# ucsdarclab/diffco

Measured on AMD Instinct MI355X. Metric: million collision-score+grad evals/sec, 7-DoF FK-kernel, 2k supports, higher is better.
Workload: dtype f32

## Files before the change

### diffco_amd/csrc/score_kernel.h

```cpp
#pragma once
#include <hip/hip_runtime.h>
#include <type_traits>
#include <stdint.h>
#include "fk_device.h"

namespace dcx {

enum { KF_RQ2 = 0,
       KF_POLY1 = 1,
       KF_GEN = 2 };

enum { MODE_SCORE = 0,
       MODE_GRAD_ROW = 1,
       MODE_GRAD_UP = 2 };

struct ScoreArgs {
    const float* rows;
    const float* centre;
    const FkProg* fk;
    const float* q;
    const float* upstream;
    float* score;
    float* grad;
    int64_t B;
// ... 125 lines not shown
#ifndef DCX_PAIR2_LOADS
#define DCX_PAIR2_LOADS 1
#endif
#ifndef DCX_LOAD_GROUPS
#define DCX_LOAD_GROUPS 1
#endif

template <int KF, bool CLAMPED = false>
__device__ __forceinline__ void kernel_eval(float d2, const ScoreArgs& a, float& val, float& g) {
    if constexpr (KF == KF_RQ2) {
        const float t = fmaf(0.5f * a.kp0, d2, 1.0f);
        const float u = __builtin_amdgcn_rcpf(t);
        val = u * u;
        g = (-2.0f * a.kp0) * (val * u);
    } else if constexpr (KF == KF_POLY1) {
        const float d2c = CLAMPED ? d2 : fmaxf(d2, 1e-30f);
        const float ri = __builtin_amdgcn_rsqf(d2c);
        val = d2c * ri;
        g = ri;
    } else {
        if (a.kind == DCX_K_RQ) {
            const float p = a.kp1;
            const float t = fmaf(a.kp0 / p, d2, 1.0f);
            val = powf(t, -p);
            g = (-2.0f * a.kp0) * val * __builtin_amdgcn_rcpf(t);
        } else if (a.kind == DCX_K_POLY) {
            const int k = (int)a.kp0;
            const float ie = 1.0f / a.kp1;
            const float d2c = fmaxf(d2, 1e-30f);
            const float ri = __builtin_amdgcn_rsqf(d2c);
            const float r = d2c * ri;
            float rk2 = (k >= 2) ? 1.0f : ri;
            for (int i = 2; i < k; ++i) rk2 *= r;
            if (k & 1) {
                val = rk2 * d2c * ie;
                g = (float)k * rk2 * ie;
            } else {
                const float lg = 0.5f * logf(d2c);
                val = rk2 * d2c * lg * ie;
                g = rk2 * fmaf((float)k, lg, 1.0f) * ie;
            }
        } else {
            const float ie2 = 1.0f / (a.kp0 * a.kp0);
            const float v2 = fmaf(d2, ie2, 1.0f);
            const float rv = __builtin_amdgcn_rsqf(v2);
            val = v2 * rv;
            g = rv * ie2;
        }
    }
}

template <int KF>
__device__ __forceinline__ float d2_seed(const ScoreArgs& a) {
    if constexpr (KF == KF_RQ2) return a.kp0;
    else return 0.0f;
}
template <int KF>
inline constexpr float kGradScale = (KF == KF_RQ2) ? -4.0f : 1.0f;
template <int KF, bool CLAMPED = false>
__device__ __forceinline__ void sweep_eval(float t, const ScoreArgs& a, float& val, float& g) {
    if constexpr (KF == KF_RQ2) {
        const float u = __builtin_amdgcn_rcpf(t);
        val = u * u;
        g = val * u;
    } else {
        kernel_eval<KF, CLAMPED>(t, a, val, g);
    }
}

struct LdsPlan {
    int fk, q, x, g, f, red, total;
};
__host__ __device__ inline LdsPlan lds_plan(int dof, int d_fk, int frame_floats, int red_slots, int acc_floats,
                                            bool alias_xg = false) {
    LdsPlan p;
    p.x = 0;
    p.g = alias_xg ? p.x : p.x + 64 * d_fk;
    p.red = p.x;
    const int end_xg = p.g + 64 * d_fk;
    const int end_red = p.red + (red_slots < 1 ? 1 : red_slots) * acc_floats * 64;
    p.q = end_xg > end_red ? end_xg : end_red;
    p.f = p.q + ((64 * dof + 3) & ~3);
    p.fk = p.f + 64 * frame_floats;
    p.total = p.fk;
    return p;
}

#ifndef DCX_MINW_SLACK
#define DCX_MINW_SLACK 0
#endif
constexpr int sweep_min_waves(int D, int CC, int KF, bool QT = false) {
    if (QT) return 4;
    const int need = 3 * D + 2 * CC + 16 + DCX_MINW_SLACK + (KF == 2 ? 40 : 0);
    return need <= 64 ? 8 : need <= 72 ? 7 : need <= 80 ? 6 : need <= 96 ? 5 : need <= 128 ? 4 : need <= 168 ? 3 : need <= 256 ? 2 : 1;
}

__device__ __forceinline__ int fresh_lane() {
    int l = (int)__builtin_amdgcn_mbcnt_hi(~0u, __builtin_amdgcn_mbcnt_lo(~0u, 0u));
    asm volatile("" : "+v"(l));
    return l;
}

template <class Args>
__device__ __forceinline__ const __attribute__((address_space(4))) Args& reload_kernargs() {
    auto p = (const __attribute__((address_space(4))) Args*)__builtin_amdgcn_kernarg_segment_ptr();
    asm volatile("" : "+s"(p));
    return *p;
}
__device__ __forceinline__ const __attribute__((address_space(4))) ScoreArgs& reload_args() { return reload_kernargs<ScoreArgs>(); }
#define DCX_COPY_DH(dst, src)          \
    do {                               \
        (dst).prog = (src).prog;       \
        (dst).n_dwords = (src).n_dwords; \
        (dst).n_steps = (src).n_steps; \
        (dst).end0 = (src).end0;       \
        (dst).n_chains = (src).n_chains; \
        (dst).pt = (src).pt;           \
        (dst).bare = (src).bare;       \
        (dst).real = (src).real;       \
        (dst).n_pt = (src).n_pt;       \
        (dst).shared_q = (src).shared_q; \
    } while (0)

__device__ __forceinline__ void row_opaque(float& u, float& v) { asm volatile("" : "+v"(u), "+v"(v)); }

#ifndef DCX_XF_TAU
#define DCX_XF_TAU 0.01f
#endif
#ifndef DCX_XF_FLUSH
#define DCX_XF_FLUSH 64
#endif

constexpr bool xf_applies(int D, int CC, int KF) {
    const int used = D + CC + (CC > 1 ? 1 : 0);
    const int parts = (4 * used <= (CC > 1 ? DCX_P0_MAX_MULTI : DCX_P0_MAX_SINGLE)) ? 0 : (used + 37) / 38;
    return (KF == KF_POLY1 || KF == KF_RQ2) && used + 1 <= 38 && parts <= 1;
}
constexpr bool spare_applies(int D, int CC, int KF) {
    return CC == 1 && (D % 4) == 0 && D >= 4 && D <= 12 && (KF == KF_POLY1 || KF == KF_RQ2) && D + 4 <= (D + 2 + 3) / 4 * 4;
}
constexpr bool p2_applies(int D, int CC, int KF) {
    return DCX_PAIR2 && DCX_PAIR2_LOADS && CC == 1 && (D % 2) == 0 && D <= DCX_PAIR2_MAX_D && 4 * (D + 1) <= DCX_P0_MAX_SINGLE &&
           (KF == KF_RQ2 || KF == KF_POLY1);
}

template <int D, int KF, int CC, int MODE, bool XF = false, int NACC = 0, bool NS = false, bool SP = false>
__device__ __forceinline__ void sweep_rows(const ScoreArgs& a, const float (&x_in)[D], const float (&up)[CC], int j0, int j1,
                                           float (&sc)[CC], float (&gx)[D]) {
    static_assert(!NS || (CC > 1 && MODE == MODE_GRAD_UP), "NS: the gradient sweep of a multi-class model");
    static_assert(!SP || (XF && spare_applies(D, CC, KF) && xf_applies(D, CC, KF)), "the spare form: expanded, one class, D = 4, 8, 12");
    float x[D];
    float e_sp = 0.0f, tot_sp = 0.0f;
    int col_sp = 0;
    if constexpr (SP) {
        const int c = a.spare - 1;
        e_sp = x_in[D - 1];
#pragma unroll
        for (int k = 0; k + 1 < D; ++k) {
            e_sp = (k == c) ? x_in[k] : e_sp;
            x[k] = (k == c) ? x_in[D - 1] : x_in[k];
        }
        x[D - 1] = 0.0f;
        col_sp = c;
        asm volatile("" : "+v"(col_sp));
    } else {
#pragma unroll
        for (int k = 0; k < D; ++k) x[k] = x_in[k];
    }
    using L = RowLayout<D, CC>;
    constexpr bool GRAD = (MODE != MODE_SCORE);
    v2f gx2[D / 2 + 1];
#pragma unroll
    for (int k = 0; k < D / 2 + 1; ++k) gx2[k] = v2f{0.0f, 0.0f};
    cfloat_ptr rows = (cfloat_ptr)(uintptr_t)a.rows;
    if constexpr (SP) {
        uint64_t rp = (uint64_t)(uintptr_t)a.rows;
        asm volatile("" : "+s"(rp));
        rows = (cfloat_ptr)(uintptr_t)rp;
    }
    constexpr int USED_DIRECT = D + CC + (CC > 1 ? 1 : 0);
    constexpr bool XFA = XF && xf_applies(D, CC, KF);
    constexpr int USED = SP ? D + 4 : USED_DIRECT + (XFA ? 1 : 0);
    constexpr int RSTRIDE = L::RS;
    constexpr int PARTS = SP ? 0 : (4 * USED <= (CC > 1 ? DCX_P0_MAX_MULTI : DCX_P0_MAX_SINGLE)) ? 0 : (USED + 37) / 38;
    constexpr bool SC2 = (CC > 1 && PARTS == 1);
    v2f sc2[CC / 2 + 1];
#pragma unroll
    for (int i = 0; i < CC / 2 + 1; ++i) sc2[i] = v2f{0.0f, 0.0f};
    auto add_scores = [&](auto weight_of, float val) __attribute__((always_inline)) {
        if constexpr (NS) {
            (void)val;
        } else if constexpr (SC2) {
            const v2f v2 = {val, val};
#pragma unroll
            for (int c = 0; c + 1 < CC; c += 2) sc2[c / 2] = __builtin_elementwise_fma(v2f{weight_of(c), weight_of(c + 1)}, v2, sc2[c / 2]);
            if constexpr (CC & 1) sc[CC - 1] = fmaf(weight_of(CC - 1), val, sc[CC - 1]);
#pragma unroll
            for (int c = 0; c + 1 < CC; c += 2) asm volatile("" : "+v"(sc2[c / 2]));
            if constexpr (CC & 1) asm volatile("" : "+v"(sc[CC - 1]));
        } else {
#pragma unroll
            for (int c = 0; c < CC; ++c) sc[c] = fmaf(weight_of(c), val, sc[c]);
        }
    };

    v2f xm[D / 2 + 1], ga[D / 2 + 1];
    float xm_tail = 0.0f, ga_tail = 0.0f, xx = 0.0f, thr = 1e-30f, asum = 0.0f;
    if constexpr (XFA) {
#pragma unroll
        for (int k = 0; k < D; ++k) xx = fmaf(x[k], x[k], xx);
        if constexpr (SP) xx = fmaf(e_sp, e_sp, xx);
        thr = fmaxf(DCX_XF_TAU * xx, 1e-30f);
#pragma unroll
        for (int k = 0; k + 1 < D; k += 2) {
            xm[k / 2] = v2f{-2.0f * x[k], -2.0f * x[k + 1]};
            ga[k / 2] = v2f{0.0f, 0.0f};
        }
        if constexpr (D & 1) xm_tail = -2.0f * x[D - 1];
        if constexpr (SP) xm[D / 2 - 1].y = 1.0f;
    }
    auto d2_x = [&](const auto& r) __attribute__((always_inline)) -> float {
        constexpr int NA = NACC > 0 ? NACC : DCX_D2_ACCS(D);
        v2f acc[NA];
        if constexpr (SP) acc[0] = v2f{xx, 0.0f};
        else acc[0] = v2f{xx + r[L::SS_OFF], 0.0f};
#pragma unroll
        for (int i = 1; i < NA; ++i) acc[i] = v2f{0.0f, 0.0f};
#pragma unroll
        for (int k = 0; k + 1 < D; k += 2) {
            const v2f rv = {r[k], r[k + 1]};
            acc[(k / 2) % NA] = __builtin_elementwise_fma(xm[k / 2], rv, acc[(k / 2) % NA]);
        }
#pragma unroll
        for (int i = 1; i < NA; ++i) acc[0] += acc[i];
        float d2 = acc[0].x + acc[0].y;
        if constexpr (D & 1) d2 = fmaf(xm_tail, r[D - 1], d2);
        if constexpr (KF == KF_POLY1) return fmaxf(d2, thr);
        else return d2;
    };
    auto coef_of = [&](const auto& r, float g) __attribute__((always_inline)) -> float {
        if constexpr (MODE == MODE_GRAD_ROW) {
            return g * r[CC > 1 ? L::WSUM_OFF : L::W_OFF];
        } else {
            float wb = 0.0f;
#pragma unroll
            for (int c = 0; c < CC; ++c) wb = fmaf(up[c], r[L::W_OFF + c], wb);
            return g * wb;
        }
    };
    auto apply_x = [&](const auto& r, float d2c, auto sign, bool keep) __attribute__((always_inline)) {
        constexpr int SIGN = decltype(sign)::value;
        float val, g;
        sweep_eval<KF, true>(d2c, a, val, g);
        if constexpr (PARTS == 1) row_opaque(val, g);
        constexpr bool SCORE_BY_COEF = (KF == KF_POLY1 && CC == 1 && MODE == MODE_GRAD_ROW);
        if constexpr (!SCORE_BY_COEF) {
            if constexpr (SIGN < 0) val = keep ? -val : 0.0f;
            add_scores([&](int c) __attribute__((always_inline)) { return r[L::W_OFF + c]; }, val);
        }
        if constexpr (GRAD) {
            float coef = coef_of(r, g);
            if constexpr (PARTS == 1) asm volatile("" : "+v"(coef));
            if constexpr (SIGN < 0) coef = keep ? -coef : 0.0f;
            if constexpr (SCORE_BY_COEF) sc[0] = fmaf(coef, d2c, sc[0]);
            const v2f c2 = {coef, coef};
#pragma unroll
            for (int k = 0; k + 1 < D; k += 2) {
                v2f rv = {r[k], r[k + 1]};
                if constexpr (SP) {
                    if (k == D - 2) rv = v2f{r[D + 2], r[D + 3]};
                }
                ga[k / 2] = __builtin_elementwise_fma(c2, rv, ga[k / 2]);
            }
            if constexpr (D & 1) ga_tail = fmaf(coef, r[D - 1], ga_tail);
            if constexpr (!SP) asum += coef;
        }
    };
    auto pair_x = [&](const auto& r) __attribute__((always_inline)) -> float {
        const float d2 = d2_x(r);
        apply_x(r, d2, std::integral_constant<int, 1>{}, true);
        return d2;
    };
    auto fix_near = [&](const auto& r, float d2c) __attribute__((always_inline)) {
        const bool nr = d2c <= thr;
        apply_x(r, d2c, std::integral_constant<int, -1>{}, nr);
        const v2f mh = {-0.5f, -0.5f};
        v2f dacc = {0.0f, 0.0f};
#pragma unroll
        for (int k = 0; k + 1 < D; k += 2) {
            const v2f rv = {r[k], r[k + 1]};
            v2f dk = xm[k / 2] * mh - rv;
            if constexpr (SP) {
                if (k == D - 2) dk.y = e_sp;
            }
            dacc = __builtin_elementwise_fma(dk, dk, dacc);
        }
        float d2d = dacc.x + dacc.y;
        if constexpr (D & 1) {
            const float dl_tail = -0.5f * xm_tail - r[D - 1];
            d2d = fmaf(dl_tail, dl_tail, d2d);
        }
        float val, g;
        kernel_eval<KF>(d2d, a, val, g);
        val = nr ? val : 0.0f;
        if constexpr (!NS) {
#pragma unroll
            for (int c = 0; c < CC; ++c) sc[c] = fmaf(r[L::W_OFF + c], val, sc[c]);
        }
        if constexpr (GRAD) {
            const float cd = nr ? -coef_of(r, g) : 0.0f;
            const v2f cd2 = {cd, cd};
#pragma unroll
            for (int k = 0; k + 1 < D; k += 2) {
                const v2f rv = {r[k], r[k + 1]};
                if (SP && k == D - 2) {
                    ga[k / 2].x = fmaf(cd, fmaf(xm[k / 2].x, -0.5f, -rv.x), ga[k / 2].x);
                    tot_sp -= cd;
                } else {
                    ga[k / 2] = __builtin_elementwise_fma(cd2, xm[k / 2] * mh - rv, ga[k / 2]);
                }
            }
            if constexpr (D & 1) ga_tail = fmaf(cd, -0.5f * xm_tail - r[D - 1], ga_tail);
        }
    };
    auto stage_x = [&](const auto& r0, const auto& r1) __attribute__((always_inline)) {
        if constexpr (KF != KF_POLY1) {
            (void)pair_x(r0);
            (void)pair_x(r1);
            return;
        }
        const auto m0 = __builtin_amdgcn_ballot_w64(pair_x(r0) <= thr);
        const auto m1 = __builtin_amdgcn_ballot_w64(pair_x(r1) <= thr);
        if (__builtin_expect((m0 | m1) != 0, 0)) {
            fix_near(r0, d2_x(r0));
            fix_near(r1, d2_x(r1));
        }
    };
    auto single_x = [&](const auto& r0) __attribute__((always_inline)) {
        if constexpr (KF != KF_POLY1) {
            (void)pair_x(r0);
            return;
        }
        if (__builtin_expect(__builtin_amdgcn_ballot_w64(pair_x(r0) <= thr) != 0, 0)) fix_near(r0, d2_x(r0));
    };
    auto flush_x = [&]() __attribute__((always_inline)) {
        if constexpr (XFA && GRAD) {
            if constexpr (SP) asum = ga[D / 2 - 1].y;
            const v2f ah = {0.5f * asum, 0.5f * asum};
#pragma unroll
            for (int k = 0; k + 1 < D; k += 2) ga[k / 2] = __builtin_elementwise_fma(xm[k / 2], ah, ga[k / 2]);
            if constexpr (D & 1) ga_tail = fmaf(xm_tail, 0.5f * asum, ga_tail);
            if constexpr (SP) {
                tot_sp += asum;
                ga[D / 2 - 1].y = 0.0f;
            }
            asum = 0.0f;
        }
    };
    auto pair = [&](const float (&r)[L::RS]) __attribute__((always_inline)) {
        float dl[D];
        float d2;
        v2f dp[D / 2 + 1];
        {
            constexpr int NA = DCX_D2_ACCS(D);
            v2f acc[NA];
            acc[0] = v2f{d2_seed<KF>(a), 0.0f};
#pragma unroll
            for (int i = 1; i < NA; ++i) acc[i] = v2f{0.0f, 0.0f};
#pragma unroll
            for (int k = 0; k + 1 < D; k += 2) {
                const v2f xv = {x[k], x[k + 1]};
                const v2f rv = {r[k], r[k + 1]};
                dp[k / 2] = xv - rv;
                acc[(k / 2) % NA] = __builtin_elementwise_fma(dp[k / 2], dp[k / 2], acc[(k / 2) % NA]);
            }
#pragma unroll
            for (int i = 1; i < NA; ++i) acc[0] += acc[i];
            d2 = acc[0].x + acc[0].y;
            if constexpr (D & 1) {
                dl[D - 1] = x[D - 1] - r[D - 1];
                d2 = fmaf(dl[D - 1], dl[D - 1], d2);
            }
        }
        float val, g;
        sweep_eval<KF>(d2, a, val, g);
        if constexpr (!NS) {
#pragma unroll
            for (int c = 0; c < CC; ++c) sc[c] = fmaf(r[L::W_OFF + c], val, sc[c]);
        }
        if constexpr (GRAD) {
            float coef;
            if constexpr (MODE == MODE_GRAD_ROW) {
                coef = g * r[CC > 1 ? L::WSUM_OFF : L::W_OFF];
            } else {
                float wb = 0.0f;
#pragma unroll
                for (int c = 0; c < CC; ++c) wb = fmaf(up[c], r[L::W_OFF + c], wb);
                coef = g * wb;
            }
            const v2f c2 = {coef, coef};
#pragma unroll
            for (int k = 0; k + 1 < D; k += 2) gx2[k / 2] = __builtin_elementwise_fma(c2, dp[k / 2], gx2[k / 2]);
            if constexpr (D & 1) gx[D - 1] = fmaf(coef, dl[D - 1], gx[D - 1]);
        }
    };
    constexpr bool P2 = !XF && p2_applies(D, CC, KF);
    static_assert(!P2 || PARTS == 0, "pair2: whole rows in the four-row budget");
    v2f gp[P2 ? D : 1];
    v2f scp = {0.0f, 0.0f};
    if constexpr (P2) {
#pragma unroll
        for (int k = 0; k < D; ++k) gp[k] = v2f{0.0f, 0.0f};
    }
    auto pair2 = [&](const float (&b)[2 * L::RS]) __attribute__((always_inline)) {
        v2f dk[D];
        v2f acc = {d2_seed<KF>(a), d2_seed<KF>(a)};
#pragma unroll
        for (int k = 0; k < D; ++k) {
            const v2f xv = {x[k], x[k]};
            const v2f rv = {b[2 * k], b[2 * k + 1]};
            dk[k] = xv - rv;
            acc = __builtin_elementwise_fma(dk[k], dk[k], acc);
        }
        v2f val, g;
        if constexpr (KF == KF_RQ2) {
            const v2f u = {__builtin_amdgcn_rcpf(acc.x), __builtin_amdgcn_rcpf(acc.y)};
            val = u * u;
            g = val * u;
        } else {
            const v2f d2c = {fmaxf(acc.x, 1e-30f), fmaxf(acc.y, 1e-30f)};
            g = v2f{__builtin_amdgcn_rsqf(d2c.x), __builtin_amdgcn_rsqf(d2c.y)};
            val = d2c * g;
        }
        const v2f w2 = {b[2 * L::W_OFF], b[2 * L::W_OFF + 1]};
        scp = __builtin_elementwise_fma(w2, val, scp);
        if constexpr (GRAD) {
            v2f coef = g * w2;
            if constexpr (MODE != MODE_GRAD_ROW) coef = coef * v2f{up[0], up[0]};
#pragma unroll
            for (int k = 0; k < D; ++k) gp[k] = __builtin_elementwise_fma(coef, dk[k], gp[k]);
        }
    };
    constexpr int USED4 = (USED + 3) / 4 * 4;
    static_assert(USED4 <= L::RS, "the row stride covers whole groups of four");
    constexpr int NLOAD = DCX_LOAD_GROUPS ? USED4 : USED;
#ifdef DCX_EXP_NO_LOADS
    int exp_real_loads = 4;
#endif
    auto load_row = [&](float (&dst)[L::RS], int j) __attribute__((always_inline)) {
        cfloat_ptr r = rows + (size_t)j * RSTRIDE;
#ifdef DCX_EXP_NO_LOADS
        if (exp_real_loads <= 0) {
#pragma unroll
            for (int e = 0; e < NLOAD; ++e) asm volatile("" : "+s"(dst[e]));
            return;
        }
        --exp_real_loads;
#endif
#pragma unroll
        for (int e = 0; e < NLOAD; ++e) {
            if (SP && e == D + 1) continue;
            dst[e] = r[e];
        }
    };

    static_assert(!XFA || PARTS <= 1, "expanded form: whole rows only");
    if constexpr (P2 && DCX_PAIR2_LOADS) {
    if (j0 < j1) {
        constexpr int R2 = 2 * L::RS;
        float ab[R2], cd[R2];
        auto load2 = [&](float (&dst)[R2], int j) __attribute__((always_inline)) {
            cfloat_ptr r = rows + (size_t)j * RSTRIDE;
#pragma unroll
            for (int e = 0; e < R2; ++e) dst[e] = r[e];
        };
        auto body2 = [&](const float (&b)[R2]) __attribute__((always_inline)) {
#pragma unroll
            for (int e = 2 * USED; e < R2; ++e) asm volatile("" ::"s"(b[e]));
            pair2(b);
        };
        const int j1e = (j1 + 1) & ~1;
        const int jl = j1e - 2;
        load2(ab, j0);
        int j = j0;
        for (; j + 3 < j1e; j += 4) {
            __builtin_amdgcn_s_waitcnt(0xC07F);
            __builtin_amdgcn_sched_barrier(0);
            load2(cd, j + 2);
            __builtin_amdgcn_sched_barrier(0);
            body2(ab);
            __builtin_amdgcn_sched_barrier(0);
            __builtin_amdgcn_s_waitcnt(0xC07F);
            __builtin_amdgcn_sched_barrier(0);
            load2(ab, (j + 4 < j1e) ? j + 4 : jl);
            __builtin_amdgcn_sched_barrier(0);
            body2(cd);
            __builtin_amdgcn_sched_barrier(0);
        }
        if (j < j1e) body2(ab);
    }
    } else if constexpr (PARTS == 0) {
    if (j0 < j1) {
        float rowA[L::RS], rowB[L::RS], rowC[L::RS], rowD[L::RS];
        const int jl = j1 - 1;
        load_row(rowA, j0);
        load_row(rowB, (j0 + 1 < j1) ? j0 + 1 : jl);
        int j = j0;
        for (; j + 3 < j1; j += 4) {
            __builtin_amdgcn_s_waitcnt(0xC07F);
            __builtin_amdgcn_sched_barrier(0);
            load_row(rowC, j + 2);
            load_row(rowD, j + 3);
            __builtin_amdgcn_sched_barrier(0);
            if constexpr (XFA) {
                stage_x(rowA, rowB);
            } else {
                pair(rowA);
                pair(rowB);
            }
            __builtin_amdgcn_sched_barrier(0);
            __builtin_amdgcn_s_waitcnt(0xC07F);
            __builtin_amdgcn_sched_barrier(0);
            load_row(rowA, (j + 4 < j1) ? j + 4 : jl);
            load_row(rowB, (j + 5 < j1) ? j + 5 : jl);
            __builtin_amdgcn_sched_barrier(0);
            if constexpr (XFA) {
                stage_x(rowC, rowD);
            } else {
                pair(rowC);
                pair(rowD);
            }
            __builtin_amdgcn_sched_barrier(0);
            if constexpr (XFA && GRAD) {
                if ((j & (DCX_XF_FLUSH - 4)) == 0) flush_x();
            }
        }
        auto one = [&](const float (&r)[L::RS]) __attribute__((always_inline)) {
            if constexpr (XFA) single_x(r);
            else pair(r);
        };
        if (j < j1) one(rowA);
        if (j + 1 < j1) one(rowB);
        if (j + 2 < j1) {
            load_row(rowC, j + 2);
            one(rowC);
        }
    }
    } else {
        constexpr int PS = ((USED + PARTS - 1) / PARTS + 3) / 4 * 4;
        constexpr int NA = DCX_D2_ACCS(D);
        float bufA[PS], bufB[PS];
        v2f acc[NA];
        v2f dp[D / 2 + 1];
        float tail_d = 0.0f;
        float wv[CC];
        float wsum = 0.0f;
        auto load_part = [&](float (&dst)[PS], int j, auto pc) __attribute__((always_inline)) {
            constexpr int P0 = decltype(pc)::value * PS;
            constexpr int LEN = (PARTS == 1 && DCX_LOAD_GROUPS) ? PS : (USED - P0 < PS) ? (USED - P0) : PS;
            cfloat_ptr r = rows + (size_t)j * RSTRIDE + P0;
#ifdef DCX_EXP_NO_LOADS
            if (exp_real_loads <= 2) {
#pragma unroll
                for (int e = 0; e < LEN; ++e) asm volatile("" : "+s"(dst[e]));
                return;
            }
            --exp_real_loads;
#endif
#pragma unroll
            for (int e = 0; e < LEN; ++e) dst[e] = r[e];
        };
        auto consume = [&](const float (&b)[PS], auto pc) __attribute__((always_inline)) {
            if constexpr (XFA) {
                single_x(b);
                return;
            }
            constexpr int P0 = decltype(pc)::value * PS;
            constexpr int LEN = (USED - P0 < PS) ? (USED - P0) : PS;
            if constexpr (decltype(pc)::value == 0) {
                acc[0] = v2f{d2_seed<KF>(a), 0.0f};
#pragma unroll
                for (int i = 1; i < NA; ++i) acc[i] = v2f{0.0f, 0.0f};
            }
#pragma unroll
            for (int e = 0; e < LEN; ++e) {
                const int g = P0 + e;
                if (g + 1 < D && (g & 1) == 0) {
                    const v2f xv = {x[g], x[g + 1]};
                    const v2f rv = {b[e], b[e + 1]};
                    dp[g / 2] = xv - rv;
                    acc[(g / 2) % NA] = __builtin_elementwise_fma(dp[g / 2], dp[g / 2], acc[(g / 2) % NA]);
                } else if (g == D - 1 && (D & 1)) {
                    tail_d = x[g] - b[e];
                } else if (g >= D && g < D + CC) {
                    wv[g - D] = b[e];
                } else if (CC > 1 && g == D + CC) {
                    wsum = b[e];
                }
            }
            if constexpr (decltype(pc)::value == PARTS - 1) {
#pragma unroll
                for (int i = 1; i < NA; ++i) acc[0] += acc[i];
                float d2 = acc[0].x + acc[0].y;
                if constexpr (D & 1) d2 = fmaf(tail_d, tail_d, d2);
                float val, g;
                sweep_eval<KF>(d2, a, val, g);
                if constexpr (PARTS == 1) row_opaque(val, g);
                add_scores([&](int c) __attribute__((always_inline)) { return wv[c]; }, val);
                if constexpr (GRAD) {
                    float coef;
                    if constexpr (MODE == MODE_GRAD_ROW) {
                        coef = g * (CC > 1 ? wsum : wv[0]);
                    } else {
                        float wb = 0.0f;
#pragma unroll
                        for (int c = 0; c < CC; ++c) wb = fmaf(up[c], wv[c], wb);
                        coef = g * wb;
                    }
                    if constexpr (PARTS == 1) asm volatile("" : "+v"(coef));
                    const v2f c2 = {coef, coef};
#pragma unroll
                    for (int k = 0; k + 1 < D; k += 2) gx2[k / 2] = __builtin_elementwise_fma(c2, dp[k / 2], gx2[k / 2]);
                    if constexpr (D & 1) gx[D - 1] = fmaf(coef, tail_d, gx[D - 1]);
                }
            }
        };
        using P0c = std::integral_constant<int, 0>;
        using P1c = std::integral_constant<int, PARTS - 1>;
        if (j0 < j1) {
            const int jl = j1 - 1;
            if constexpr (PARTS == 1) {
                static_assert(PS <= RSTRIDE, "a whole row in groups of four floats stays inside its stride");
                load_part(bufA, j0, P0c{});
                int j = j0;
                for (; j + 1 < j1; j += 2) {
                    __builtin_amdgcn_s_waitcnt(0xC07F);
                    __builtin_amdgcn_sched_barrier(0);
                    load_part(bufB, j + 1, P0c{});
                    __builtin_amdgcn_sched_barrier(0);
                    consume(bufA, P0c{});
                    __builtin_amdgcn_sched_barrier(0);
                    __builtin_amdgcn_s_waitcnt(0xC07F);
                    __builtin_amdgcn_sched_barrier(0);
                    load_part(bufA, (j + 2 < j1) ? j + 2 : jl, P0c{});
                    __builtin_amdgcn_sched_barrier(0);
                    consume(bufB, P0c{});
                    __builtin_amdgcn_sched_barrier(0);
                    if constexpr (XFA && GRAD) {
                        if ((j & (DCX_XF_FLUSH - 2)) == 0) flush_x();
                    }
                }
                if (j < j1) consume(bufA, P0c{});
            } else if constexpr (PARTS == 2) {
                load_part(bufA, j0, P0c{});
                for (int j = j0; j < j1; ++j) {
                    __builtin_amdgcn_s_waitcnt(0xC07F);
                    __builtin_amdgcn_sched_barrier(0);
                    load_part(bufB, j, P1c{});
                    __builtin_amdgcn_sched_barrier(0);
                    consume(bufA, P0c{});
                    __builtin_amdgcn_sched_barrier(0);
                    __builtin_amdgcn_s_waitcnt(0xC07F);
                    __builtin_amdgcn_sched_barrier(0);
                    load_part(bufA, (j + 1 < j1) ? j + 1 : jl, P0c{});
                    __builtin_amdgcn_sched_barrier(0);
                    consume(bufB, P1c{});
                    __builtin_amdgcn_sched_barrier(0);
                }
            } else {
                auto step = [&](auto self, auto uc, int j) __attribute__((always_inline)) -> void {
                    constexpr int U = decltype(uc)::value;
                    constexpr int NU = U + 1;
                    __builtin_amdgcn_s_waitcnt(0xC07F);
                    __builtin_amdgcn_sched_barrier(0);
                    {
                        const int jr = j + NU / PARTS;
                        const int row = jr < j1 ? jr : jl;
                        if constexpr (NU % 2 == 0) load_part(bufA, row, std::integral_constant<int, NU % PARTS>{});
                        else load_part(bufB, row, std::integral_constant<int, NU % PARTS>{});
                    }
                    __builtin_amdgcn_sched_barrier(0);
                    if constexpr (U % 2 == 0) consume(bufA, std::integral_constant<int, U % PARTS>{});
                    else consume(bufB, std::integral_constant<int, U % PARTS>{});
                    __builtin_amdgcn_sched_barrier(0);
                    if constexpr (U + 1 < 2 * PARTS) self(self, std::integral_constant<int, U + 1>{}, j);
                };
                load_part(bufA, j0, P0c{});
                int j = j0;
                for (; j + 1 < j1; j += 2) step(step, P0c{}, j);
                if (j < j1) {
                    auto tail = [&](auto self, auto pc) __attribute__((always_inline)) -> void {
                        constexpr int P = decltype(pc)::value;
                        __builtin_amdgcn_s_waitcnt(0xC07F);
                        __builtin_amdgcn_sched_barrier(0);
                        if constexpr (P + 1 < PARTS) {
                            if constexpr ((P + 1) % 2 == 0) load_part(bufA, j, std::integral_constant<int, P + 1>{});
                            else load_part(bufB, j, std::integral_constant<int, P + 1>{});
                        }
                        __builtin_amdgcn_sched_barrier(0);
                        if constexpr (P % 2 == 0) consume(bufA, pc);
                        else consume(bufB, pc);
                        __builtin_amdgcn_sched_barrier(0);
                        if constexpr (P + 1 < PARTS) self(self, std::integral_constant<int, P + 1>{});
                    };
                    tail(tail, P0c{});
                }
            }
        }
    }

    if constexpr (XFA && GRAD) {
        flush_x();
        if constexpr (SP) {
            const int c = __builtin_amdgcn_readfirstlane(col_sp);
            const float gl = e_sp * tot_sp;
            float gsw = gl;
#pragma unroll
            for (int k = 0; k + 1 < D; ++k) {
                const float h = (k & 1) ? ga[k / 2].y : ga[k / 2].x;
                gsw = (k == c) ? -h : gsw;
                gx[k] += (k == c) ? gl : -h;
            }
            gx[D - 1] += gsw;
        } else {
#pragma unroll
        for (int k = 0; k + 1 < D; k += 2) {
            gx[k] -= ga[k / 2].x;
            gx[k + 1] -= ga[k / 2].y;
        }
        if constexpr (D & 1) gx[D - 1] -= ga_tail;
        }
    } else {
#pragma unroll
        for (int k = 0; k + 1 < D; k += 2) {
            gx[k] += gx2[k / 2].x;
            gx[k + 1] += gx2[k / 2].y;
        }
        if constexpr (P2) {
            sc[0] += scp.x + scp.y;
            if constexpr (GRAD) {
#pragma unroll
                for (int k = 0; k < D; ++k) gx[k] += gp[k].x + gp[k].y;
            }
        }
    }
    if constexpr (SC2) {
#pragma unroll
        for (int c = 0; c + 1 < CC; c += 2) {
            sc[c] += sc2[c / 2].x;
            sc[c + 1] += sc2[c / 2].y;
        }
    }
    if constexpr (GRAD && kGradScale<KF> != 1.0f) {
#pragma unroll
        for (int k = 0; k < D; ++k) gx[k] *= kGradScale<KF>;
    }
}

constexpr int kQtSlices = 4;
constexpr bool qt_applies(int D, int CC, int KF, int MODE) {
    return (D == 12 || D == 24) && CC == 1 && (MODE == 1  || MODE == 0 ) && KF != 2 ;
}
template <int D, int KF, bool GRAD>
__device__ __forceinline__ void sweep_rows_lds(const ScoreArgs& a, const float (&x)[D], const float* slice, int per, float& sc0,
                                               float (&gx)[D]) {
    static_assert(D % 4 == 0, "rows are read as whole float4s");
    using L = RowLayout<D, 1>;
    v2f g2[D / 2];
#pragma unroll
    for (int k = 0; k < D / 2; ++k) g2[k] = v2f{0.0f, 0.0f};
    typedef float v4f_t __attribute__((ext_vector_type(4)));
    auto load_row = [&](float (&r)[D + 1], int jj) __attribute__((always_inline)) {
        const float* p = slice + (size_t)jj * L::RS;
#pragma unroll
        for (int q = 0; q < D / 4; ++q) {
            const v4f_t v = *reinterpret_cast<const v4f_t*>(p + 4 * q);
            r[4 * q] = v.x; r[4 * q + 1] = v.y; r[4 * q + 2] = v.z; r[4 * q + 3] = v.w;
        }
        r[D] = p[L::W_OFF];
    };
    auto pair = [&](const float (&r)[D + 1]) __attribute__((always_inline)) {
        v2f dp[D / 2];
        constexpr int NA = DCX_D2_ACCS(D);
        v2f acc[NA];
        acc[0] = v2f{d2_seed<KF>(a), 0.0f};
#pragma unroll
        for (int i = 1; i < NA; ++i) acc[i] = v2f{0.0f, 0.0f};
#pragma unroll
        for (int k = 0; k + 1 < D; k += 2) {
            const v2f xv = {x[k], x[k + 1]};
            const v2f rv = {r[k], r[k + 1]};
            dp[k / 2] = xv - rv;
            acc[(k / 2) % NA] = __builtin_elementwise_fma(dp[k / 2], dp[k / 2], acc[(k / 2) % NA]);
        }
#pragma unroll
        for (int i = 1; i < NA; ++i) acc[0] += acc[i];
        const float d2 = acc[0].x + acc[0].y;
        float val, g;
        sweep_eval<KF>(d2, a, val, g);
        sc0 = fmaf(r[D], val, sc0);
        if constexpr (GRAD) {
            const float coef = g * r[D];
            const v2f c2 = {coef, coef};
#pragma unroll
            for (int k = 0; k + 1 < D; k += 2) g2[k / 2] = __builtin_elementwise_fma(c2, dp[k / 2], g2[k / 2]);
        }
    };
    float ra[D + 1], rb[D + 1];
    load_row(ra, 0);
    int jj = 0;
    for (; jj + 2 <= per; jj += 2) {
        load_row(rb, jj + 1);
        pair(ra);
        load_row(ra, jj + 2 < per ? jj + 2 : jj + 1);
        pair(rb);
    }
    if (jj < per) pair(ra);
    if constexpr (GRAD) {
#pragma unroll
        for (int k = 0; k + 1 < D; k += 2) {
            gx[k] += g2[k / 2].x * kGradScale<KF>;
            gx[k + 1] += g2[k / 2].y * kGradScale<KF>;
        }
    }
}

template <int ACC, int E0 = 0, int E1 = ACC>
__device__ __forceinline__ void fold_partial_rows(float* sRed, int wave, int lane, int nw) {
    auto fold_rows = [&](auto nwc) __attribute__((always_inline)) {
        constexpr int NWC = decltype(nwc)::value;
// ... 529 lines not shown
```

Baseline: 795.3.

## Add lean SP fast path computing paired distances before near-check

```diff
diff --git a/diffco_amd/csrc/score_kernel.h b/diffco_amd/csrc/score_kernel.h
--- a/diffco_amd/csrc/score_kernel.h
+++ b/diffco_amd/csrc/score_kernel.h
@@ -451,6 +451,7 @@
         }
         float val, g;
         kernel_eval<KF>(d2d, a, val, g);
+        if constexpr (SP && KF == KF_POLY1) val = (d2d == d2d) ? val : d2d;
         val = nr ? val : 0.0f;
         if constexpr (!NS) {
 #pragma unroll
@@ -472,7 +473,81 @@
             if constexpr (D & 1) ga_tail = fmaf(cd, -0.5f * xm_tail - r[D - 1], ga_tail);
         }
     };
-    auto stage_x = [&](const auto& r0, const auto& r1) __attribute__((always_inline)) {
+    auto d2_raw2 = [&](const auto& r0, const auto& r1) __attribute__((always_inline)) -> v2f {
+        constexpr int NA = NACC > 0 ? NACC : DCX_D2_ACCS(D);
+        v2f a0[NA], a1[NA];
+        a0[0] = a1[0] = v2f{xx, 0.0f};
+#pragma unroll
+        for (int i = 1; i < NA; ++i) a0[i] = a1[i] = v2f{0.0f, 0.0f};
+#pragma unroll
+        for (int k = 0; k + 1 < D; k += 2) {
+            a0[(k / 2) % NA] = __builtin_elementwise_fma(xm[k / 2], v2f{r0[k], r0[k + 1]}, a0[(k / 2) % NA]);
+            a1[(k / 2) % NA] = __builtin_elementwise_fma(xm[k / 2], v2f{r1[k], r1[k + 1]}, a1[(k / 2) % NA]);
+        }
+#pragma unroll
+        for (int i = 1; i < NA; ++i) {
+            a0[0] += a0[i];
+            a1[0] += a1[i];
+        }
+        return v2f{a0[0].x + a0[0].y, a1[0].x + a1[0].y};
+    };
+    auto fold_x = [&](const auto& r, float d2, float val, float coef) __attribute__((always_inline)) {
+        constexpr bool SCORE_BY_COEF = (KF == KF_POLY1 && MODE == MODE_GRAD_ROW);
+        if constexpr (!SCORE_BY_COEF) sc[0] = fmaf(r[L::W_OFF], val, sc[0]);
+        if constexpr (GRAD) {
+            if constexpr (SCORE_BY_COEF) sc[0] = fmaf(coef, d2, sc[0]);
+            const v2f c2 = {coef, coef};
+#pragma unroll
+            for (int k = 0; k + 1 < D; k += 2) {
+                const v2f rv = (k == D - 2) ? v2f{r[D + 2], r[D + 3]} : v2f{r[k], r[k + 1]};
+                ga[k / 2] = __builtin_elementwise_fma(c2, rv, ga[k / 2]);
+            }
+        }
+    };
+    auto quarter2 = [&](v2f d2) __attribute__((always_inline)) -> v2f {
+        if constexpr (KF == KF_RQ2) return v2f{__builtin_amdgcn_rcpf(d2.x), __builtin_amdgcn_rcpf(d2.y)};
+        else return v2f{__builtin_amdgcn_rsqf(d2.x), __builtin_amdgcn_rsqf(d2.y)};
+    };
+    auto lean_stage_x = [&](const auto& r0, const auto& r1, v2f d2, v2f q2) __attribute__((always_inline)) {
+        v2f val2, g2, coef2 = {0.0f, 0.0f};
+        if constexpr (KF == KF_RQ2) {
+            val2 = q2 * q2;
+            g2 = val2 * q2;
+        } else {
+            g2 = q2;
+            val2 = d2 * g2;
+        }
+        if constexpr (GRAD) {
+            v2f w2 = {r0[L::W_OFF], r1[L::W_OFF]};
+            if constexpr (MODE != MODE_GRAD_ROW) w2 = v2f{fmaf(up[0], w2.x, 0.0f), fmaf(up[0], w2.y, 0.0f)};
+            coef2 = g2 * w2;
+        }
+        fold_x(r0, d2.x, val2.x, coef2.x);
+        fold_x(r1, d2.y, val2.y, coef2.y);
+    };
+    auto stage_x = [&](const auto& r0, const auto& r1, const auto& n0, const auto& n1) __attribute__((always_inline)) {
+        if constexpr (SP) {
+            const v2f d2 = d2_raw2(r0, r1);
+            if constexpr (KF == KF_POLY1) {
+                const auto m0 = __builtin_amdgcn_ballot_w64(!(d2.x > thr));
+                const auto m1 = __builtin_amdgcn_ballot_w64(!(d2.y > thr));
+                auto near = m0 | m1;
+                v2f q2 = quarter2(d2);
+                asm volatile("" : "+v"(q2));
+                if (__builtin_expect(near != 0, 0)) {
+                    (void)pair_x(r0);
+                    (void)pair_x(r1);
+                    fix_near(r0, d2_x(r0));
+                    fix_near(r1, d2_x(r1));
+                    asm volatile("" ::"s"(n0[D + 2]), "s"(n0[D + 3]), "s"(n1[D + 2]), "s"(n1[D + 3]));
+                }
+                asm volatile("" : "+s"(near));
+                if (__builtin_expect(near == 0, 1)) lean_stage_x(r0, r1, d2, q2);
+                return;
+            }
+            lean_stage_x(r0, r1, d2, quarter2(d2));
+            return;
+        }
         if constexpr (KF != KF_POLY1) {
             (void)pair_x(r0);
             (void)pair_x(r1);
@@ -488,6 +563,17 @@
     auto single_x = [&](const auto& r0) __attribute__((always_inline)) {
         if constexpr (KF != KF_POLY1) {
             (void)pair_x(r0);
+            return;
+        }
+        if constexpr (SP) {
+            const float d2 = d2_raw2(r0, r0).x;
+            auto near = __builtin_amdgcn_ballot_w64(!(d2 > thr));
+            if (__builtin_expect(near != 0, 0)) {
+                (void)pair_x(r0);
+                fix_near(r0, d2_x(r0));
+            }
+            asm volatile("" : "+s"(near));
+            if (__builtin_expect(near == 0, 1)) apply_x(r0, d2, std::integral_constant<int, 1>{}, true);
             return;
         }
         if (__builtin_expect(__builtin_amdgcn_ballot_w64(pair_x(r0) <= thr) != 0, 0)) fix_near(r0, d2_x(r0));
@@ -662,7 +748,7 @@
             load_row(rowD, j + 3);
             __builtin_amdgcn_sched_barrier(0);
             if constexpr (XFA) {
-                stage_x(rowA, rowB);
+                stage_x(rowA, rowB, rowC, rowD);
             } else {
                 pair(rowA);
                 pair(rowB);
@@ -674,7 +760,7 @@
             load_row(rowB, (j + 5 < j1) ? j + 5 : jl);
             __builtin_amdgcn_sched_barrier(0);
             if constexpr (XFA) {
-                stage_x(rowC, rowD);
+                stage_x(rowC, rowD, rowA, rowB);
             } else {
                 pair(rowC);
                 pair(rowD);
```

New measurement: 814.7 (median of 6 runs). 1.02x the previous value.
